# tenstack/batch-scheduler

Measured on NVIDIA H100. Metric: pod_x_node_fit_evals_per_sec, higher is better.
Workload: dtype int64

## Files before the change

batch-scheduler_b200/csrc/common.cuh:

```cuda
#pragma once
#include <cuda_runtime.h>
#include <stdint.h>

#include "../../include/bsched.h"

namespace bsk {

constexpr int LANE_CPU = 0, LANE_MEM = 1, LANE_EPH = 2, LANE_PODS = 3;
constexpr int64_t ABSENT_LEFT = (int64_t)1 << 61;
constexpr int64_t UNCHECKED_REQ = -((int64_t)1 << 61);
constexpr int32_t ABSENT_LEFT32 = 1 << 29;
constexpr int32_t UNCHECKED_REQ32 = -(1 << 29);
constexpr int FIT_CAP_LOG2 = 27;
constexpr int64_t NARROW_LIMIT = ((int64_t)1 << (FIT_CAP_LOG2 - 1)) - 1;
constexpr int32_t ABSENT_LEFTS = (1 << 30) - 1;
constexpr int32_t UNCHECKED_REQS = -((1 << 30) - 1);
constexpr int64_t SCALED_LIMIT = (int64_t)1 << 29;
struct LaneMap {
  uint8_t wide[BS_MAX_LANES];
  uint8_t narrow[BS_MAX_LANES];
  uint8_t scaled[BS_MAX_LANES];
  uint8_t sunit[BS_MAX_LANES];
  uint8_t sshift[BS_MAX_LANES];
  uint32_t sclamp[BS_MAX_LANES];
  uint32_t LW, LN, LS;
};
constexpr int NODE_TILE = 512;
constexpr int FIT_WARPS = 8;
constexpr int FIT_THREADS = (FIT_WARPS + 1) * 32;
constexpr int FIT_MIN_BLOCKS = 2;
constexpr int PODS_PER_WARP = 4;
constexpr int PODS_PER_CTA = FIT_WARPS * PODS_PER_WARP;
constexpr int TILE_WORDS = NODE_TILE / 32;
static_assert(TILE_WORDS <= 32 && 32 % TILE_WORDS == 0, "a 32-word bitmap line is a whole number of tiles");
constexpr int TILES_PER_LINE = 32 / TILE_WORDS;
constexpr int KEY_BITS = 4;
static_assert((1 << KEY_BITS) == TILE_WORDS, "the best-node key holds a word index of the tile in KEY_BITS bits");
static_assert(FIT_CAP_LOG2 + KEY_BITS <= 31, "best-node key: score (27 bits) + word index must fit 31 bits");
constexpr int FIT_STAGES = 2;
static_assert(TILE_WORDS % 4 == 0, "the fit kernel sweeps a tile 4 words at a time");
constexpr int FIT_NB = 2;
using ColBits = uint16_t;
static_assert(sizeof(ColBits) * 8 == TILE_WORDS, "one class bit per ballot word of a tile");

}
```

batch-scheduler_b200/csrc/fit.cuh:

```cuda
#pragma once
#include "common.cuh"

namespace bsk {

__device__ __forceinline__ uint32_t smem_u32(const void* p) {
  return (uint32_t)__cvta_generic_to_shared(p);
}
__device__ __forceinline__ void mbar_init(uint64_t* bar, uint32_t count) {
  asm volatile("mbarrier.init.shared::cta.b64 [%0], %1;" ::"r"(smem_u32(bar)), "r"(count));
}
__device__ __forceinline__ void mbar_expect_tx(uint64_t* bar, uint32_t bytes) {
  asm volatile("mbarrier.arrive.expect_tx.shared::cta.b64 _, [%0], %1;" ::"r"(smem_u32(bar)), "r"(bytes)
               : "memory");
}
__device__ __forceinline__ void mbar_arrive(uint64_t* bar) {
  asm volatile("mbarrier.arrive.shared::cta.b64 _, [%0];" ::"r"(smem_u32(bar)) : "memory");
}
__device__ __forceinline__ void mbar_wait(uint64_t* bar, uint32_t parity) {
  asm volatile(
      "{\n"
      ".reg .pred p;\n"
      "WAIT_%=:\n"
      "mbarrier.try_wait.parity.shared::cta.b64 p, [%0], %1;\n"
      "@p bra DONE_%=;\n"
      "bra WAIT_%=;\n"
      "DONE_%=:\n"
      "}\n" ::"r"(smem_u32(bar)),
      "r"(parity)
      : "memory");
}
__device__ __forceinline__ void tma_bulk_g2s(void* dst_smem, const void* src_gmem, uint32_t bytes,
                                             uint64_t* bar) {
  asm volatile(
      "cp.async.bulk.shared::cluster.global.mbarrier::complete_tx::bytes [%0], [%1], %2, [%3];" ::"r"(
          smem_u32(dst_smem)),
      "l"(src_gmem), "r"(bytes), "r"(smem_u32(bar))
      : "memory");
}
__device__ __forceinline__ uint64_t l2_evict_first() {
  uint64_t pol;
  asm volatile("createpolicy.fractional.L2::evict_first.b64 %0, 1.0;" : "=l"(pol));
  return pol;
}
__device__ __forceinline__ void tma_bulk_s2g(void* dst_gmem, uint32_t src_smem, uint32_t bytes, uint64_t pol) {
  asm volatile("cp.async.bulk.global.shared::cta.bulk_group.L2::cache_hint [%0], [%1], %2, %3;" ::"l"(dst_gmem),
               "r"(src_smem), "r"(bytes), "l"(pol)
               : "memory");
}
__device__ __forceinline__ void bulk_commit() { asm volatile("cp.async.bulk.commit_group;" ::: "memory"); }
template <int N>
__device__ __forceinline__ void bulk_wait_read() { asm volatile("cp.async.bulk.wait_group.read %0;" ::"n"(N) : "memory"); }
__device__ __forceinline__ void fence_async_smem() { asm volatile("fence.proxy.async.shared::cta;" ::: "memory"); }

__device__ __forceinline__ int64_t min64(int64_t a, int64_t b) { return a < b ? a : b; }
__device__ __forceinline__ int32_t hi32(int64_t v) {
  int32_t lo, hi;
  asm("mov.b64 {%0, %1}, %2;" : "=r"(lo), "=r"(hi) : "l"(v));
  (void)lo;
  return hi;
}
__device__ __forceinline__ uint32_t lo32(int64_t v) {
  int32_t lo, hi;
  asm("mov.b64 {%0, %1}, %2;" : "=r"(lo), "=r"(hi) : "l"(v));
  (void)hi;
  return (uint32_t)lo;
}
__device__ __forceinline__ void sts_u32(uint32_t saddr, uint32_t v) {
  asm volatile("st.shared.u32 [%0], %1;" ::"r"(saddr), "r"(v));
}
__device__ __forceinline__ void sts_v2u32(uint32_t saddr, uint32_t lo, uint32_t hi) {
  asm volatile("st.shared.v2.u32 [%0], {%1, %2};" ::"r"(saddr), "r"(lo), "r"(hi));
}
__device__ __forceinline__ void sts_u64(uint32_t saddr, long long v) {
  asm volatile("st.shared.u64 [%0], %1;" ::"r"(saddr), "l"(v));
}

struct FitArgs {
  const int64_t* left_w;
  const int32_t* left_n;
  const ColBits* classfit;
  const int64_t* req;
  const uint32_t* req_present;
  const uint32_t* fit_class;
  LaneMap lm;
  uint32_t* feasible_count;
  int32_t* best_node;
  int64_t* best_score;
  uint32_t* fit_bitmap;
  int64_t* score;
  uint64_t left_w_pitch, left_n_pitch;
  uint64_t score_pitch;
  uint32_t bitmap_pitch;
  uint32_t P, N, Npad, W;
  uint32_t n_full, tail_split;
  unsigned long long* best_packed;
  int32_t* topk_node;
  int64_t* topk_score;
  uint32_t topk_k;
};

template <bool NARROW> struct BestT { using type = int64_t; };
template <> struct BestT<true> { using type = int32_t; };

enum { FIT_OUT_NONE = 0, FIT_OUT_BITMAP = 1, FIT_OUT_SCORE = 2, FIT_OUT_TOPK = 3 };

template <typename S>
__device__ __forceinline__ S topk_insert(S* __restrict__ ls_p, int32_t* __restrict__ ln_p, uint32_t K, uint32_t cb,
                                         S s, int32_t n0 , uint32_t lane) {
  S ls = ls_p[lane];
  int32_t ln = ln_p[lane];
#pragma unroll 1
  do {
    const uint32_t src = __ffs(cb) - 1;
    cb &= cb - 1;
    const S cs = __shfl_sync(0xffffffffu, s, src);
    const int32_t cn = n0 + (int32_t)src;
    const uint32_t pos = __popc(__ballot_sync(0xffffffffu, ls > cs || (ls == cs && ln < cn)));
    if (pos < K) {
      const S us = __shfl_up_sync(0xffffffffu, ls, 1);
      const int32_t un = __shfl_up_sync(0xffffffffu, ln, 1);
      if (lane == pos) { ls = cs; ln = cn; }
      else if (lane > pos) { ls = us; ln = un; }
    }
  } while (cb);
  ls_p[lane] = ls;
  ln_p[lane] = ln;
  return __shfl_sync(0xffffffffu, ls, K - 1);
}

template <int LW, int LN, int LS, int OUT, int RN>
__device__ __forceinline__ void fit_tile(const FitArgs& a, const int64_t* __restrict__ tlw,
                                         const int32_t* __restrict__ tln,
                                         const int64_t (&rqw)[PODS_PER_WARP][LW > 0 ? LW : 1],
                                         const int32_t (&rqn)[PODS_PER_WARP][LN + LS > 0 ? LN + LS : 1],
                                         const ColBits (&colbits)[PODS_PER_WARP], int R0, uint32_t slab ,
                                         uint32_t* s_words, uint32_t wbase , uint32_t node_base, uint32_t lane,
                                         typename BestT<(LN > 0)>::type (&best_s)[PODS_PER_WARP],
                                         int32_t (&best_n)[PODS_PER_WARP], int32_t (&kb)[PODS_PER_WARP],
                                         uint32_t (&cnt)[PODS_PER_WARP],
                                         typename BestT<(LN > 0)>::type* tks, int32_t* tkn ,
                                         typename BestT<(LN > 0)>::type (&thr)[PODS_PER_WARP]) {
  constexpr bool SCORE = OUT == FIT_OUT_SCORE;
  constexpr bool TOPK = OUT == FIT_OUT_TOPK;
  constexpr bool WORDS = OUT == FIT_OUT_BITMAP || SCORE;
  using S = typename BestT<(LN > 0)>::type;
  static_assert(!SCORE || RN == 1, "a staging slab holds one matrix row");
  const int64_t* tpw = tlw + lane;
  const int32_t* tpn = tln + lane;
  int32_t node = (int32_t)(node_base + lane);
  uint32_t wp = smem_u32(s_words) + wbase * 4;
  uint32_t sp = slab + lane * 8;
  int32_t jrem = TILE_WORDS - 1;
#pragma unroll 1
  for (int jb = 0; jb < TILE_WORDS; jb += 4) {
#pragma unroll
    for (int jj = 0; jj < 4; ++jj) {
      int64_t lfw[LW > 0 ? LW : 1];
      int32_t lfn[LN + LS > 0 ? LN + LS : 1];
#pragma unroll
      for (int d = 0; d < LW; ++d) lfw[d] = tpw[d * NODE_TILE + jj * 32];
#pragma unroll
      for (int d = 0; d < LN + LS; ++d) lfn[d] = tpn[d * NODE_TILE + jj * 32];
#pragma unroll
      for (int i = 0; i < RN; ++i) {
        const int r = R0 + i;
        if (LN > 0) {
          int32_t t = lfn[0] - rqn[r][0];
#pragma unroll
          for (int d = 1; d < LN; ++d) t = min(t, lfn[d] - rqn[r][d]);
          uint32_t m32 = (uint32_t)t;
          int32_t sgn = t;
#pragma unroll
          for (int d = 0; d < LS; ++d) {
            const int32_t x = min(lfn[LN + d] - rqn[r][LN + d], (int32_t)a.lm.sclamp[d]);
            sgn |= x;
            m32 = min(m32, (uint32_t)x << a.lm.sshift[d]);
          }
#pragma unroll
          for (int d = 0; d < LW; ++d) {
            const int64_t w = lfw[d] - rqw[r][d];
            const int32_t whi = hi32(w);
            sgn |= whi;
            m32 = min(m32, whi != 0 ? 0xffffffffu : lo32(w));
          }
          const bool fit = (sgn >= 0) && ((colbits[r] >> (jb + jj)) & 1u);
          if (WORDS) sts_u32(wp + (r * 32 + jj) * 4, __ballot_sync(0xffffffffu, fit));
          else if (fit) ++cnt[r];
          if (TOPK && a.fit_bitmap) sts_u32(wp + (r * 32 + jj) * 4, __ballot_sync(0xffffffffu, fit));
          const int32_t key = (int32_t)(m32 << KEY_BITS) + (jrem - jj);
          if (!TOPK && fit) kb[r] = max(kb[r], key);
          if (SCORE) sts_v2u32(sp + jj * 32 * 8, fit ? m32 : 0u, fit ? 0u : 0x80000000u);
          if (TOPK) {
            const uint32_t cb = __ballot_sync(0xffffffffu, fit && (int32_t)m32 > thr[r]);
            if (cb) thr[r] = topk_insert<S>(tks + r * 32, tkn + r * 32, a.topk_k, cb, (int32_t)m32, node + jj * 32 - (int32_t)lane, lane);
          }
        } else {
          int64_t m = lfw[0] - rqw[r][0];
#pragma unroll
          for (int d = 1; d < LW; ++d) m = min64(m, lfw[d] - rqw[r][d]);
          const bool fit = (hi32(m) >= 0) && ((colbits[r] >> (jb + jj)) & 1u);
          if (WORDS) sts_u32(wp + (r * 32 + jj) * 4, __ballot_sync(0xffffffffu, fit));
          else if (fit) ++cnt[r];
          if (TOPK && a.fit_bitmap) sts_u32(wp + (r * 32 + jj) * 4, __ballot_sync(0xffffffffu, fit));
          if (!TOPK && fit && m > best_s[r]) { best_s[r] = m; best_n[r] = node + jj * 32; }
          if (SCORE) sts_u64(sp + jj * 32 * 8, fit ? (long long)m : (long long)INT64_MIN);
          if (TOPK) {
            const uint32_t cb = __ballot_sync(0xffffffffu, fit && m > thr[r]);
            if (cb) thr[r] = topk_insert<S>(tks + r * 32, tkn + r * 32, a.topk_k, cb, m, node + jj * 32 - (int32_t)lane, lane);
          }
        }
      }
    }
    tpw += 128;
    tpn += 128;
    node += 128;
    jrem -= 4;
    wp += 16;
    sp += 128 * 8;
  }
}

__host__ __device__ constexpr size_t fit_tile_bytes(int LW, int LN, int LS) {
  return (size_t)NODE_TILE * (8 * LW + 4 * (LN + LS));
}
__host__ __device__ constexpr size_t fit_slab_bytes() { return (size_t)NODE_TILE * 8; }
__host__ __device__ constexpr size_t fit_topk_bytes() { return (size_t)PODS_PER_CTA * BS_TOPK_MAX * 12; }
static_assert(BS_TOPK_MAX == 32, "a top-K list holds one entry per lane");
__host__ __device__ constexpr size_t fit_smem_front(int LW, int LN, int LS) {
  size_t b = FIT_STAGES * fit_tile_bytes(LW, LN, LS) + (size_t)PODS_PER_CTA * (8 * LW + 4 * (LN + LS));
  b = (b + 7) & ~(size_t)7;
  b += 2 * FIT_STAGES * sizeof(uint64_t) + (size_t)PODS_PER_CTA * 32 * sizeof(uint32_t);
  return (b + 127) & ~(size_t)127;
}
__host__ __device__ constexpr size_t fit_smem_total(int LW, int LN, int LS, int out) {
  return fit_smem_front(LW, LN, LS) + (out == FIT_OUT_SCORE  ? (size_t)FIT_WARPS * FIT_NB * fit_slab_bytes()
                                       : out == FIT_OUT_TOPK ? fit_topk_bytes()
                                                             : 0);
}
constexpr size_t FIT_SMEM_MAX = 227 * 1024;

template <int LW, int LN, int LS, int OUT>
__global__ void __launch_bounds__(FIT_THREADS, FIT_MIN_BLOCKS) gang_fit_kernel(FitArgs a) {
  constexpr bool SCORE = OUT == FIT_OUT_SCORE;
  constexpr bool TOPK = OUT == FIT_OUT_TOPK;
  constexpr bool WORDS = OUT == FIT_OUT_BITMAP || SCORE;
  extern __shared__ __align__(128) unsigned char smem_raw[];
  constexpr size_t STAGE_BYTES = fit_tile_bytes(LW, LN, LS);
  constexpr int LNS = LN + LS;
  unsigned char* s_tile = smem_raw;
  int64_t* s_req_w = reinterpret_cast<int64_t*>(smem_raw + FIT_STAGES * STAGE_BYTES);
  int32_t* s_req_n = reinterpret_cast<int32_t*>(s_req_w + PODS_PER_CTA * LW);
  uint64_t* s_bar = reinterpret_cast<uint64_t*>(
      (reinterpret_cast<uintptr_t>(s_req_n + PODS_PER_CTA * LNS) + 7) & ~(uintptr_t)7);
  uint64_t* s_full = s_bar;
  uint64_t* s_empty = s_bar + FIT_STAGES;
  uint32_t* s_words_all = reinterpret_cast<uint32_t*>(s_bar + 2 * FIT_STAGES);

  const uint32_t tid = threadIdx.x, lane = tid & 31, wid = tid >> 5;
  uint32_t* s_words = s_words_all + wid * PODS_PER_WARP * 32;
  uint32_t unit = blockIdx.x, piece = 0, npieces = 1;
  if (blockIdx.x >= a.n_full) {
    const uint32_t tl = blockIdx.x - a.n_full;
    unit = a.n_full + tl / a.tail_split;
    piece = tl % a.tail_split;
    npieces = a.tail_split;
  }
  const uint32_t pod0 = unit * PODS_PER_CTA;
  const uint32_t wpod0 = pod0 + wid * PODS_PER_WARP;
  const uint32_t n_tiles = a.Npad / NODE_TILE;
  const uint32_t n_lines = (n_tiles + TILES_PER_LINE - 1) / TILES_PER_LINE;
  const uint32_t tile_lo = min(n_tiles, (n_lines * piece / npieces) * TILES_PER_LINE);
  const uint32_t tile_hi = min(n_tiles, (n_lines * (piece + 1) / npieces) * TILES_PER_LINE);

  if (tid == 0) {
    for (int st = 0; st < FIT_STAGES; ++st) {
      mbar_init(&s_full[st], 1);
      mbar_init(&s_empty[st], FIT_WARPS);
    }
    asm volatile("fence.mbarrier_init.release.cluster;" ::: "memory");
  }
  for (uint32_t i = tid; i < PODS_PER_CTA * (LW + LNS); i += FIT_THREADS) {
    const uint32_t pl = i / (LW + LNS), k = i % (LW + LNS);
    const uint32_t p = pod0 + pl;
    const bool is_w = k < (uint32_t)LW;
    const uint32_t kn = k - LW;
    const uint32_t d = is_w ? a.lm.wide[k] : (kn < (uint32_t)LN ? a.lm.narrow[kn] : a.lm.scaled[kn - LN]);
    int64_t v = 0;
    bool present = true;
    if (p < a.P) {
      present = d < 4 || ((a.req_present[p] >> d) & 1u);
      v = present ? a.req[(size_t)d * a.P + p] : 0;
    }
    if (is_w) s_req_w[pl * LW + k] = present ? v : UNCHECKED_REQ;
    else if (kn < (uint32_t)LN) s_req_n[pl * LNS + kn] = present ? (int32_t)v : UNCHECKED_REQ32;
    else s_req_n[pl * LNS + kn] = present ? (int32_t)(v >> a.lm.sunit[kn - LN]) : UNCHECKED_REQS;
  }
  __syncthreads();
  auto issue = [&](uint32_t tile, uint32_t stage) {
    mbar_expect_tx(&s_full[stage], (uint32_t)STAGE_BYTES);
    unsigned char* dst = s_tile + stage * STAGE_BYTES;
    const unsigned char* src_w = reinterpret_cast<const unsigned char*>(a.left_w) + (uint64_t)tile * (NODE_TILE * 8);
    const unsigned char* src_n = reinterpret_cast<const unsigned char*>(a.left_n) + (uint64_t)tile * (NODE_TILE * 4);
#pragma unroll
    for (int d = 0; d < LW; ++d)
      tma_bulk_g2s(dst + (size_t)d * NODE_TILE * 8, src_w + (uint64_t)d * a.left_w_pitch, NODE_TILE * 8,
                   &s_full[stage]);
#pragma unroll
    for (int d = 0; d < LNS; ++d)
      tma_bulk_g2s(dst + (size_t)LW * NODE_TILE * 8 + (size_t)d * NODE_TILE * 4,
                   src_n + (uint64_t)d * a.left_n_pitch, NODE_TILE * 4, &s_full[stage]);
  };
  if (wid == FIT_WARPS) {
    if (lane == 0) {
      for (uint32_t tile = tile_lo; tile < tile_hi; ++tile) {
        const uint32_t st = (tile - tile_lo) % FIT_STAGES, use = (tile - tile_lo) / FIT_STAGES;
        if (use > 0) mbar_wait(&s_empty[st], (use - 1) & 1);
        issue(tile, st);
      }
    }
    return;
  }

  const bool want_bitmap = a.fit_bitmap != nullptr;
  uint32_t cnt[PODS_PER_WARP];
  typename BestT<(LN > 0)>::type best_s[PODS_PER_WARP];
  int32_t best_n[PODS_PER_WARP];
  int32_t kb[PODS_PER_WARP], kthr[PODS_PER_WARP];
  typename BestT<(LN > 0)>::type thr[PODS_PER_WARP];
  int64_t rqw[PODS_PER_WARP][LW > 0 ? LW : 1];
  int32_t rqn[PODS_PER_WARP][LNS > 0 ? LNS : 1];
  uint32_t coff[PODS_PER_WARP];
  typename BestT<(LN > 0)>::type* tks =
      reinterpret_cast<typename BestT<(LN > 0)>::type*>(smem_raw + fit_smem_front(LW, LN, LS)) + wid * PODS_PER_WARP * 32;
  int32_t* tkn = reinterpret_cast<int32_t*>(smem_raw + fit_smem_front(LW, LN, LS) + (size_t)PODS_PER_CTA * 32 * 8) +
                 wid * PODS_PER_WARP * 32;
#pragma unroll
  for (int r = 0; r < PODS_PER_WARP; ++r) {
    cnt[r] = 0; best_n[r] = -1; kb[r] = -1; kthr[r] = 0; thr[r] = -1;
    if (TOPK) { tks[r * 32 + lane] = -1; tkn[r * 32 + lane] = -1; }
    best_s[r] = LN > 0 ? (typename BestT<(LN > 0)>::type)(-1) : (typename BestT<(LN > 0)>::type)INT64_MIN;
    const uint32_t p = wpod0 + r;
    coff[r] = (p < a.P ? a.fit_class[p] : 0u) * n_tiles * 32 + lane;
#pragma unroll
    for (int d = 0; d < LW; ++d) rqw[r][d] = s_req_w[(wid * PODS_PER_WARP + r) * LW + d];
#pragma unroll
    for (int d = 0; d < LNS; ++d) rqn[r][d] = s_req_n[(wid * PODS_PER_WARP + r) * LNS + d];
  }
  const uint32_t slab0 = smem_u32(smem_raw + fit_smem_front(LW, LN, LS)) + wid * (uint32_t)(FIT_NB * fit_slab_bytes());
  int64_t* srow = SCORE ? a.score + (size_t)wpod0 * a.score_pitch : nullptr;

  uint32_t stage = 0, phase = 0, sb = 0, nseg = 0;
  ColBits colnext[PODS_PER_WARP];
#pragma unroll
  for (int r = 0; r < PODS_PER_WARP; ++r) colnext[r] = __ldg(a.classfit + coff[r] + min(tile_lo, n_tiles - 1) * 32);
  for (uint32_t tile = tile_lo; tile < tile_hi; ++tile) {
    ColBits colbits[PODS_PER_WARP];
    const uint32_t tnext = tile + 1 < tile_hi ? tile + 1 : tile;
#pragma unroll
    for (int r = 0; r < PODS_PER_WARP; ++r) {
      colbits[r] = colnext[r];
      colnext[r] = __ldg(a.classfit + coff[r] + tnext * 32);
    }
    mbar_wait(&s_full[stage], phase);
    const int64_t* tlw = reinterpret_cast<const int64_t*>(s_tile + stage * STAGE_BYTES);
    const int32_t* tln = reinterpret_cast<const int32_t*>(s_tile + stage * STAGE_BYTES + (size_t)LW * NODE_TILE * 8);
    const uint32_t node_base = tile * NODE_TILE;
    const uint32_t wbase = (tile % TILES_PER_LINE) * TILE_WORDS;
    if constexpr (SCORE) {
#pragma unroll
      for (int r = 0; r < PODS_PER_WARP; ++r) {
        const uint32_t slab = slab0 + sb * (uint32_t)fit_slab_bytes();
        if (nseg >= (uint32_t)FIT_NB) {
          if (lane == 0) bulk_wait_read<FIT_NB - 1>();
          __syncwarp();
        }
        fit_tile<LW, LN, LS, OUT, 1>(a, tlw, tln, rqw, rqn, colbits, r, slab, s_words, wbase, node_base, lane, best_s,
                                     best_n, kb, cnt, tks, tkn, thr);
        fence_async_smem();
        __syncwarp();
        if (lane == 0) {
          if (node_base < (uint32_t)a.score_pitch) {
            const uint32_t cols = min((uint32_t)NODE_TILE, (uint32_t)a.score_pitch - node_base);
            tma_bulk_s2g(srow + (size_t)r * a.score_pitch + node_base, slab, cols * 8, l2_evict_first());
          }
          bulk_commit();
        }
        ++nseg;
        if (++sb == FIT_NB) sb = 0;
      }
    } else {
      fit_tile<LW, LN, LS, OUT, PODS_PER_WARP>(a, tlw, tln, rqw, rqn, colbits, 0, 0, s_words, wbase, node_base, lane,
                                               best_s, best_n, kb, cnt, tks, tkn, thr);
    }
    if (LN > 0 && !TOPK) {
#pragma unroll
      for (int r = 0; r < PODS_PER_WARP; ++r) {
        if (kb[r] >= kthr[r]) {
          best_s[r] = kb[r] >> KEY_BITS;
          best_n[r] = (int32_t)(node_base + lane) + (TILE_WORDS - 1 - (kb[r] & (TILE_WORDS - 1))) * 32;
          kthr[r] = (best_s[r] + 1) << KEY_BITS;
        }
        kb[r] = -1;
      }
    }
    __syncwarp();
    if (lane == 0) mbar_arrive(&s_empty[stage]);
    if ((WORDS || (TOPK && want_bitmap)) && ((tile + 1) % TILES_PER_LINE == 0 || tile + 1 == tile_hi)) {
      const uint32_t line = tile / TILES_PER_LINE;
      const uint32_t valid = (tile % TILES_PER_LINE + 1) * TILE_WORDS;
      if (lane < valid) {
#pragma unroll
        for (int r = 0; r < PODS_PER_WARP; ++r) {
          const uint32_t w = s_words[r * 32 + lane];
          if (WORDS) cnt[r] += __popc(w);
          if (want_bitmap) a.fit_bitmap[(size_t)(wpod0 + r) * a.bitmap_pitch + line * 32 + lane] = w;
        }
      }
    }
    __syncwarp();
    if (++stage == FIT_STAGES) { stage = 0; phase ^= 1; }
  }
  if (SCORE && lane == 0) bulk_wait_read<0>();
  if (TOPK && lane < a.topk_k) {
#pragma unroll
    for (int r = 0; r < PODS_PER_WARP; ++r) {
      const size_t o = (size_t)(wpod0 + r) * a.topk_k + lane;
      const int32_t n = tkn[r * 32 + lane];
      a.topk_node[o] = n;
      a.topk_score[o] = n < 0 ? INT64_MIN : (int64_t)tks[r * 32 + lane];
    }
  }

#pragma unroll
  for (int k = 0; k < PODS_PER_WARP; ++k) {
    int32_t n = TOPK ? tkn[k * 32] : best_n[k];
    int64_t s = n < 0 ? INT64_MIN : TOPK ? (int64_t)tks[k * 32] : (int64_t)best_s[k];
    uint32_t c = cnt[k];
    for (int o = 16; o; o >>= 1) {
      const int64_t os = __shfl_xor_sync(0xffffffffu, s, o);
      const int32_t on = __shfl_xor_sync(0xffffffffu, n, o);
      c += __shfl_xor_sync(0xffffffffu, c, o);
      if (on >= 0 && (n < 0 || os > s || (os == s && on < n))) { s = os; n = on; }
    }
    const uint32_t p = wpod0 + k;
    if (p < a.P && lane == 0) {
      if (npieces == 1) {
        a.feasible_count[p] = c;
        a.best_node[p] = n;
        a.best_score[p] = s;
      } else {
        if (c) atomicAdd(&a.feasible_count[p], c);
        if (n >= 0) atomicMax(&a.best_packed[p], ((unsigned long long)(uint32_t)(s + 1) << 32) | (uint32_t)(~(uint32_t)n));
      }
    }
  }
}

static __global__ void fit_unpack_kernel(const unsigned long long* __restrict__ packed, uint32_t p0, uint32_t P,
                                         int32_t* __restrict__ best_node, int64_t* __restrict__ best_score) {
  const uint32_t p = p0 + blockIdx.x * blockDim.x + threadIdx.x;
  if (p >= P) return;
  const unsigned long long v = packed[p];
  if (v == 0) { best_node[p] = -1; best_score[p] = INT64_MIN; return; }
  best_node[p] = (int32_t)(~(uint32_t)v);
  best_score[p] = (int64_t)(v >> 32) - 1;
}
constexpr uint32_t FIT_TAIL_SPLIT = 8;

}

namespace bsk {
using FitFn = cudaError_t (*)(const FitArgs&, uint32_t units, cudaStream_t, uint32_t* launches, cudaEvent_t ev_a, cudaEvent_t ev_b);
constexpr int FIT_MAX_LN = 8;
constexpr int FIT_N_SLICES = FIT_MAX_LN + 1;
struct FitWS { int lw, ls; };
constexpr FitWS FIT_WS_COMBOS[] = {{0, 0}, {1, 0}, {2, 0}, {3, 0}, {4, 0}, {0, 1}, {0, 2}, {0, 3}, {1, 1}, {1, 2}, {2, 1}};
constexpr int FIT_N_WS = sizeof(FIT_WS_COMBOS) / sizeof(FIT_WS_COMBOS[0]);
inline bool fit_variant_exists(uint32_t LW, uint32_t LN, uint32_t LS) {
  if (LN == 0) return LS == 0 && LW >= 4 && LW <= BS_MAX_LANES;
  if (LN > (uint32_t)FIT_MAX_LN || LW + LN + LS < 4 || LW + LN + LS > BS_MAX_LANES) return false;
  for (int i = 0; i < FIT_N_WS; ++i)
    if ((uint32_t)FIT_WS_COMBOS[i].lw == LW && (uint32_t)FIT_WS_COMBOS[i].ls == LS) return true;
  return false;
}
FitFn fit_lookup_slice0(uint32_t LW, uint32_t LN, uint32_t LS, int out);
FitFn fit_lookup_slice1(uint32_t LW, uint32_t LN, uint32_t LS, int out);
FitFn fit_lookup_slice2(uint32_t LW, uint32_t LN, uint32_t LS, int out);
FitFn fit_lookup_slice3(uint32_t LW, uint32_t LN, uint32_t LS, int out);
FitFn fit_lookup_slice4(uint32_t LW, uint32_t LN, uint32_t LS, int out);
FitFn fit_lookup_slice5(uint32_t LW, uint32_t LN, uint32_t LS, int out);
FitFn fit_lookup_slice6(uint32_t LW, uint32_t LN, uint32_t LS, int out);
FitFn fit_lookup_slice7(uint32_t LW, uint32_t LN, uint32_t LS, int out);
FitFn fit_lookup_slice8(uint32_t LW, uint32_t LN, uint32_t LS, int out);
inline FitFn fit_lookup(uint32_t LW, uint32_t LN, uint32_t LS, int out) {
  switch (LN) {
    case 0: return fit_lookup_slice0(LW, LN, LS, out);
    case 1: return fit_lookup_slice1(LW, LN, LS, out);
    case 2: return fit_lookup_slice2(LW, LN, LS, out);
    case 3: return fit_lookup_slice3(LW, LN, LS, out);
    case 4: return fit_lookup_slice4(LW, LN, LS, out);
    case 5: return fit_lookup_slice5(LW, LN, LS, out);
    case 6: return fit_lookup_slice6(LW, LN, LS, out);
    case 7: return fit_lookup_slice7(LW, LN, LS, out);
    case 8: return fit_lookup_slice8(LW, LN, LS, out);
  }
  return nullptr;
}
}
```

batch-scheduler_b200/csrc/fit_inst.cu:

```cuda
#include <algorithm>

#include "fit.cuh"

#ifndef BS_FIT_SLICE
#error "compile with -DBS_FIT_SLICE=<0..8>"
#endif

namespace bsk {
namespace {

template <int LW, int LN, int LS, int OUT>
cudaError_t launch_fit_t(const FitArgs& a0, uint32_t units, cudaStream_t s, uint32_t* launches, cudaEvent_t ev_a, cudaEvent_t ev_b) {
  constexpr size_t smem = fit_smem_total(LW, LN, LS, OUT);
  static_assert(smem <= FIT_SMEM_MAX, "the fit kernel's shared memory exceeds what one CTA may use");
  cudaError_t er = cudaFuncSetAttribute(gang_fit_kernel<LW, LN, LS, OUT>, cudaFuncAttributeMaxDynamicSharedMemorySize,
                                        (int)smem);
  if (er != cudaSuccess) return er;
  FitArgs a = a0;
  a.n_full = units;
  a.tail_split = 1;
  if (LN > 0 && OUT != FIT_OUT_TOPK && a.best_packed && units) {
    int per_sm = 0, dev = 0, sms = 0;
    if (cudaOccupancyMaxActiveBlocksPerMultiprocessor(&per_sm, gang_fit_kernel<LW, LN, LS, OUT>, FIT_THREADS, smem) == cudaSuccess &&
        cudaGetDevice(&dev) == cudaSuccess && cudaDeviceGetAttribute(&sms, cudaDevAttrMultiProcessorCount, dev) == cudaSuccess &&
        per_sm > 0 && sms > 0) {
      const uint32_t slots = (uint32_t)per_sm * (uint32_t)sms;
      const uint32_t n_tiles = a.Npad / NODE_TILE, n_lines = (n_tiles + TILES_PER_LINE - 1) / TILES_PER_LINE;
      const uint32_t n_full = units / slots * slots, tail = units - n_full;
      const uint32_t split = std::min<uint32_t>(FIT_TAIL_SPLIT, n_lines);
      if (tail && split > 1 && tail * 10 < slots * 9) {
        a.n_full = n_full;
        a.tail_split = split;
      }
    }
  }
  const uint32_t tail_units = units - a.n_full;
  if (a.tail_split > 1) {
    const uint32_t p0 = a.n_full * PODS_PER_CTA;
    if (p0 < a.P) {
      er = cudaMemsetAsync(a.feasible_count + p0, 0, (size_t)(a.P - p0) * 4, s);
      if (er == cudaSuccess) er = cudaMemsetAsync(a.best_packed + p0, 0, (size_t)(a.P - p0) * 8, s);
      if (er != cudaSuccess) return er;
    }
  }
  if (ev_a) cudaEventRecord(ev_a, s);
  gang_fit_kernel<LW, LN, LS, OUT><<<a.n_full + tail_units * a.tail_split, FIT_THREADS, smem, s>>>(a);
  if (ev_b) cudaEventRecord(ev_b, s);
  if (launches) *launches = 1;
  if (a.tail_split > 1) {
    const uint32_t p0 = a.n_full * PODS_PER_CTA;
    if (p0 < a.P) {
      fit_unpack_kernel<<<(a.P - p0 + 255) / 256, 256, 0, s>>>(a.best_packed, p0, a.P, a.best_node, a.best_score);
      if (launches) *launches = 2;
    }
  }
  return cudaGetLastError();
}

template <int LW, int LN, int LS>
FitFn pick(int out) {
  switch (out) {
    case FIT_OUT_SCORE: return launch_fit_t<LW, LN, LS, FIT_OUT_SCORE>;
    case FIT_OUT_BITMAP: return launch_fit_t<LW, LN, LS, FIT_OUT_BITMAP>;
    case FIT_OUT_TOPK: return launch_fit_t<LW, LN, LS, FIT_OUT_TOPK>;
  }
  return launch_fit_t<LW, LN, LS, FIT_OUT_NONE>;
}

}

#define BS_CAT2(a, b) a##b
#define BS_CAT(a, b) BS_CAT2(a, b)

FitFn BS_CAT(fit_lookup_slice, BS_FIT_SLICE)(uint32_t LW, uint32_t LN, uint32_t LS, int score) {
#if BS_FIT_SLICE == 0
  if (LN != 0 || LS != 0) return nullptr;
  switch (LW) {
    case 4: return pick<4, 0, 0>(score);
    case 6: return pick<6, 0, 0>(score);
    case 7: return pick<7, 0, 0>(score);
    case 8: return pick<8, 0, 0>(score);
    case 9: return pick<9, 0, 0>(score);
    case 10: return pick<10, 0, 0>(score);
    case 11: return pick<11, 0, 0>(score);
    case 12: return pick<12, 0, 0>(score);
    case 13: return pick<13, 0, 0>(score);
    case 14: return pick<14, 0, 0>(score);
    case 15: return pick<15, 0, 0>(score);
    case 16: return pick<16, 0, 0>(score);
    case 5: return pick<5, 0, 0>(score);
  }
  return nullptr;
#else
  constexpr int N = BS_FIT_SLICE;
  if (LN != (uint32_t)N || !fit_variant_exists(LW, LN, LS)) return nullptr;
  const uint32_t key = LW * 8 + LS;
  switch (key) {
#define BS_CASE(lw, ls)                                                        \
  case lw * 8 + ls:                                                            \
    if constexpr (lw + N + ls >= 4) return pick<lw, N, ls>(score); else break;
    BS_CASE(0, 0) BS_CASE(1, 0) BS_CASE(2, 0) BS_CASE(3, 0) BS_CASE(4, 0) BS_CASE(0, 1) BS_CASE(0, 2) BS_CASE(0, 3)
    BS_CASE(1, 1) BS_CASE(1, 2) BS_CASE(2, 1)
#undef BS_CASE
  }
  return nullptr;
#endif
}

}
```

profiles/microbench/store_pattern2.cu:

```cuda
#include <cstdio>
#include <cstdint>
#include <cstring>
#include <cuda_runtime.h>

__device__ __forceinline__ uint32_t smem_u32(const void* p) { return (uint32_t)__cvta_generic_to_shared(p); }
__device__ __forceinline__ void bulk_s2g(void* gdst, const void* ssrc, uint32_t bytes) {
  asm volatile("cp.async.bulk.global.shared::cta.bulk_group [%0], [%1], %2;" ::"l"(gdst), "r"(smem_u32(ssrc)), "r"(bytes)
               : "memory");
}
__device__ __forceinline__ void bulk_commit() { asm volatile("cp.async.bulk.commit_group;" ::: "memory"); }
template <int N>
__device__ __forceinline__ void bulk_wait_read() { asm volatile("cp.async.bulk.wait_group.read %0;" ::"n"(N) : "memory"); }
__device__ __forceinline__ void fence_async_smem() { asm volatile("fence.proxy.async.shared::cta;" ::: "memory"); }

__global__ void fill(long long* p, size_t n) {
  for (size_t i = blockIdx.x * (size_t)blockDim.x + threadIdx.x; i < n; i += (size_t)gridDim.x * blockDim.x) __stcs(p + i, 7ll);
}

template <int R>
__global__ void rows(long long* out, int P, int N) {
  const int lane = threadIdx.x & 31, wid = threadIdx.x >> 5, nw = blockDim.x >> 5;
  const int row0 = (blockIdx.x * nw + wid) * R;
  for (int base = 0; base < N; base += 512)
    for (int j = 0; j < 16; ++j)
#pragma unroll
      for (int r = 0; r < R; ++r) {
        const int n = base + j * 32 + lane;
        if (row0 + r < P && n < N) __stcs(out + (size_t)(row0 + r) * N + n, (long long)(n + r));
      }
}

template <int R>
__global__ void rowsv2(long long* out, int P, int N) {
  const int lane = threadIdx.x & 31, wid = threadIdx.x >> 5, nw = blockDim.x >> 5;
  const int row0 = (blockIdx.x * nw + wid) * R;
  for (int base = 0; base < N; base += 512)
    for (int j = 0; j < 8; ++j)
#pragma unroll
      for (int r = 0; r < R; ++r) {
        const int n = base + j * 64 + lane * 2;
        if (row0 + r < P && n + 1 < N)
          __stcs(reinterpret_cast<longlong2*>(out + (size_t)(row0 + r) * N + n), make_longlong2(n + r, n + r + 1));
      }
}

template <int R, int T, int NB, int WARPS>
__global__ void __launch_bounds__(WARPS * 32) tma(long long* out, int P, int N) {
  extern __shared__ __align__(128) unsigned char smem[];
  const int lane = threadIdx.x & 31, wid = threadIdx.x >> 5;
  long long* slab = reinterpret_cast<long long*>(smem) + (size_t)wid * NB * R * T;
  const int row0 = (blockIdx.x * WARPS + wid) * R;
  if (row0 >= P) return;
  int it = 0;
  for (int base = 0; base < N; base += T, ++it) {
    long long* s = slab + (size_t)(it % NB) * R * T;
    if (it >= NB) {
      if (lane == 0) bulk_wait_read<NB - 1>();
      __syncwarp();
    }
    const int cols = min(T, N - base);
#pragma unroll 4
    for (int j = 0; j < T / 32; ++j)
#pragma unroll
      for (int r = 0; r < R; ++r) s[r * T + j * 32 + lane] = (long long)(base + j * 32 + lane + r);
    fence_async_smem();
    __syncwarp();
    if (lane == 0) {
#pragma unroll
      for (int r = 0; r < R; ++r)
        if (row0 + r < P) bulk_s2g(out + (size_t)(row0 + r) * N + base, s + r * T, (uint32_t)cols * 8);
      bulk_commit();
    }
  }
  if (lane == 0) bulk_wait_read<0>();
}

template <int R, int T, int NB, int WARPS>
__global__ void __launch_bounds__(WARPS * 32) tmacta(long long* out, int P, int N) {
  extern __shared__ __align__(128) unsigned char smem[];
  const int lane = threadIdx.x & 31, wid = threadIdx.x >> 5;
  constexpr int ROWS = R * WARPS;
  long long* slab0 = reinterpret_cast<long long*>(smem);
  const int row0 = blockIdx.x * ROWS;
  int it = 0;
  for (int base = 0; base < N; base += T, ++it) {
    long long* s = slab0 + (size_t)(it % NB) * ROWS * T;
    if (it >= NB) {
      if (threadIdx.x == 0) bulk_wait_read<NB - 1>();
      __syncthreads();
    }
    const int cols = min(T, N - base);
#pragma unroll 4
    for (int j = 0; j < T / 32; ++j)
#pragma unroll
      for (int r = 0; r < R; ++r) s[(wid * R + r) * T + j * 32 + lane] = (long long)(base + j * 32 + lane + r);
    fence_async_smem();
    __syncthreads();
    if (threadIdx.x == 0) {
      for (int r = 0; r < ROWS; ++r)
        if (row0 + r < P) bulk_s2g(out + (size_t)(row0 + r) * N + base, s + r * T, (uint32_t)cols * 8);
      bulk_commit();
    }
  }
  if (threadIdx.x == 0) bulk_wait_read<0>();
}

template <class F>
float timeit(F f) {
  cudaEvent_t a, b;
  cudaEventCreate(&a); cudaEventCreate(&b);
  for (int i = 0; i < 3; ++i) f();
  float best = 1e9f, sum = 0;
  for (int i = 0; i < 10; ++i) {
    cudaEventRecord(a); f(); cudaEventRecord(b); cudaEventSynchronize(b);
    float ms; cudaEventElapsedTime(&ms, a, b); best = ms < best ? ms : best; sum += ms;
  }
  cudaEventDestroy(a); cudaEventDestroy(b);
  printf("   [avg %.3f]", sum / 10);
  return best;
}

static long long* d;
static const int P = 100000, N = 10000;
static void rep(const char* name, float ms) {
  cudaError_t e = cudaGetLastError();
  printf(" %-28s %.3f ms  %.0f GB/s  %s\n", name, ms, (double)P * N * 8 / ms / 1e6, e == cudaSuccess ? "" : cudaGetErrorString(e));
}

template <int R, int T, int NB, int WARPS>
void run_tma(const char* name, size_t smem_pad = 0) {
  const size_t smem = smem_pad ? smem_pad : (size_t)WARPS * NB * R * T * 8;
  cudaFuncSetAttribute(tma<R, T, NB, WARPS>, cudaFuncAttributeMaxDynamicSharedMemorySize, (int)smem);
  int occ = 0;
  cudaOccupancyMaxActiveBlocksPerMultiprocessor(&occ, tma<R, T, NB, WARPS>, WARPS * 32, smem);
  const int grid = (P + R * WARPS - 1) / (R * WARPS);
  cudaMemset(d, 0xff, 1 << 20);
  float ms = timeit([&] { tma<R, T, NB, WARPS><<<grid, WARPS * 32, smem>>>(d, P, N); });
  long long h[4];
  cudaMemcpy(h, d + 5, 8, cudaMemcpyDeviceToHost);
  cudaMemcpy(h + 1, d + (size_t)(R > 1 ? 1 : 0) * N + 9999, 8, cudaMemcpyDeviceToHost);
  cudaMemcpy(h + 2, d + (size_t)(P - 1) * N + 4097, 8, cudaMemcpyDeviceToHost);
  const bool ok = h[0] == 5 && h[1] == 9999 + (R > 1 ? 1 : 0) && h[2] == 4097 + ((P - 1) % R);
  char buf[96];
  snprintf(buf, sizeof buf, "%s occ=%d smem=%zuK %s", name, occ, smem >> 10, ok ? "ok" : "BAD");
  rep(buf, ms);
}
template <int R, int T, int NB, int WARPS>
void run_tmacta(const char* name) {
  const size_t smem = (size_t)WARPS * NB * R * T * 8;
  cudaFuncSetAttribute(tmacta<R, T, NB, WARPS>, cudaFuncAttributeMaxDynamicSharedMemorySize, (int)smem);
  int occ = 0;
  cudaOccupancyMaxActiveBlocksPerMultiprocessor(&occ, tmacta<R, T, NB, WARPS>, WARPS * 32, smem);
  const int grid = (P + R * WARPS - 1) / (R * WARPS);
  float ms = timeit([&] { tmacta<R, T, NB, WARPS><<<grid, WARPS * 32, smem>>>(d, P, N); });
  long long h[4];
  cudaMemcpy(h, d + 5, 8, cudaMemcpyDeviceToHost);
  cudaMemcpy(h + 2, d + (size_t)(P - 1) * N + 4097, 8, cudaMemcpyDeviceToHost);
  const bool ok = h[0] == 5 && h[2] == 4097 + ((P - 1) % R);
  char buf[96];
  snprintf(buf, sizeof buf, "%s occ=%d smem=%zuK %s", name, occ, smem >> 10, ok ? "ok" : "BAD");
  rep(buf, ms);
}

int main(int argc, char** argv) {
  const size_t n = (size_t)P * N;
  cudaMalloc(&d, n * 8 + (1 << 20));
  if (argc > 1 && !strcmp(argv[1], "occ2")) {
    constexpr size_t FIT_SMEM = 90880;
    for (int k = 0; k < 3; ++k) {
      run_tma<4, 128, 2, 8>("tma R4 T128 NB2 W8 pad", FIT_SMEM);
      run_tma<1, 512, 2, 8>("tma R1 T512 NB2 W8 pad", FIT_SMEM);
      run_tma<2, 256, 2, 8>("tma R2 T256 NB2 W8 pad", FIT_SMEM);
    }
    rep("memset", timeit([&] { cudaMemsetAsync(d, 1, n * 8); }));
    cudaError_t e = cudaDeviceSynchronize();
    printf("status: %s\n", cudaGetErrorString(e));
    return 0;
  }
  rep("fill", timeit([&] { fill<<<132 * 8, 256>>>(d, n); }));
  rep("memset", timeit([&] { cudaMemsetAsync(d, 1, n * 8); }));
  rep("rows<4> (round-1 pattern)", timeit([&] { rows<4><<<(P + 31) / 32, 256>>>(d, P, N); }));
  rep("rows<1> 8 rows/CTA", timeit([&] { rows<1><<<(P + 7) / 8, 256>>>(d, P, N); }));
  rep("rows<1> 16 rows/CTA", timeit([&] { rows<1><<<(P + 15) / 16, 512>>>(d, P, N); }));
  rep("rowsv2<4> 16B stores", timeit([&] { rowsv2<4><<<(P + 31) / 32, 256>>>(d, P, N); }));
  rep("rowsv2<1> 16B stores", timeit([&] { rowsv2<1><<<(P + 7) / 8, 256>>>(d, P, N); }));
  run_tma<4, 128, 2, 8>("tma R4 T128 NB2 W8");
  run_tma<4, 256, 2, 8>("tma R4 T256 NB2 W8");
  run_tma<4, 512, 1, 8>("tma R4 T512 NB1 W8");
  run_tma<2, 256, 2, 8>("tma R2 T256 NB2 W8");
  run_tma<2, 512, 2, 8>("tma R2 T512 NB2 W8");
  run_tma<1, 512, 2, 8>("tma R1 T512 NB2 W8");
  run_tma<1, 1024, 2, 8>("tma R1 T1024 NB2 W8");
  run_tma<4, 256, 3, 4>("tma R4 T256 NB3 W4");
  run_tma<4, 128, 4, 8>("tma R4 T128 NB4 W8");
  run_tma<4, 64, 4, 8>("tma R4 T64 NB4 W8");
  run_tmacta<4, 128, 2, 8>("tmacta R4 T128 NB2 W8");
  run_tmacta<4, 256, 2, 8>("tmacta R4 T256 NB2 W8");
  run_tmacta<4, 64, 3, 8>("tmacta R4 T64 NB3 W8");
  cudaError_t e = cudaDeviceSynchronize();
  printf("status: %s\n", cudaGetErrorString(e));
  return 0;
}
```

Measured before the change: 353.4 billion.

## Give score-mode fit warps one pod each and launch four times more CTAs

In score-output mode each warp now handles a single pod instead of four, so a CTA covers 8 pods and the grid is scaled up to match. Each warp streams one contiguous matrix row through its staging slabs instead of interleaving four rows per node tile. The aim is more CTAs and warps sharing the score-matrix store bandwidth, with long sequential bulk stores per row. In exchange, every node tile is loaded into shared memory four times as often across the grid, since fewer pods reuse each staged tile. A microbenchmark comparing the two row-store patterns is also added.

```diff
diff --git a/batch-scheduler_b200/csrc/common.cuh b/batch-scheduler_b200/csrc/common.cuh
--- a/batch-scheduler_b200/csrc/common.cuh
+++ b/batch-scheduler_b200/csrc/common.cuh
@@ -31,6 +31,9 @@
 constexpr int FIT_MIN_BLOCKS = 2;
 constexpr int PODS_PER_WARP = 4;
 constexpr int PODS_PER_CTA = FIT_WARPS * PODS_PER_WARP;
+constexpr int SCORE_PODS_PER_WARP = 1;
+constexpr int SCORE_PODS_PER_CTA = FIT_WARPS * SCORE_PODS_PER_WARP;
+static_assert(PODS_PER_CTA % SCORE_PODS_PER_CTA == 0, "score-mode CTAs tile the padded rows");
 constexpr int TILE_WORDS = NODE_TILE / 32;
 static_assert(TILE_WORDS <= 32 && 32 % TILE_WORDS == 0, "a 32-word bitmap line is a whole number of tiles");
 constexpr int TILES_PER_LINE = 32 / TILE_WORDS;
diff --git a/batch-scheduler_b200/csrc/fit.cuh b/batch-scheduler_b200/csrc/fit.cuh
--- a/batch-scheduler_b200/csrc/fit.cuh
+++ b/batch-scheduler_b200/csrc/fit.cuh
@@ -128,23 +128,23 @@
   return __shfl_sync(0xffffffffu, ls, K - 1);
 }
 
-template <int LW, int LN, int LS, int OUT, int RN>
+template <int LW, int LN, int LS, int OUT, int PW>
 __device__ __forceinline__ void fit_tile(const FitArgs& a, const int64_t* __restrict__ tlw,
                                          const int32_t* __restrict__ tln,
-                                         const int64_t (&rqw)[PODS_PER_WARP][LW > 0 ? LW : 1],
-                                         const int32_t (&rqn)[PODS_PER_WARP][LN + LS > 0 ? LN + LS : 1],
-                                         const ColBits (&colbits)[PODS_PER_WARP], int R0, uint32_t slab ,
+                                         const int64_t (&rqw)[PW][LW > 0 ? LW : 1],
+                                         const int32_t (&rqn)[PW][LN + LS > 0 ? LN + LS : 1],
+                                         const ColBits (&colbits)[PW], uint32_t slab ,
                                          uint32_t* s_words, uint32_t wbase , uint32_t node_base, uint32_t lane,
-                                         typename BestT<(LN > 0)>::type (&best_s)[PODS_PER_WARP],
-                                         int32_t (&best_n)[PODS_PER_WARP], int32_t (&kb)[PODS_PER_WARP],
-                                         uint32_t (&cnt)[PODS_PER_WARP],
+                                         typename BestT<(LN > 0)>::type (&best_s)[PW],
+                                         int32_t (&best_n)[PW], int32_t (&kb)[PW],
+                                         uint32_t (&cnt)[PW],
                                          typename BestT<(LN > 0)>::type* tks, int32_t* tkn ,
-                                         typename BestT<(LN > 0)>::type (&thr)[PODS_PER_WARP]) {
+                                         typename BestT<(LN > 0)>::type (&thr)[PW]) {
   constexpr bool SCORE = OUT == FIT_OUT_SCORE;
   constexpr bool TOPK = OUT == FIT_OUT_TOPK;
   constexpr bool WORDS = OUT == FIT_OUT_BITMAP || SCORE;
   using S = typename BestT<(LN > 0)>::type;
-  static_assert(!SCORE || RN == 1, "a staging slab holds one matrix row");
+  static_assert(!SCORE || PW == 1, "a staging slab holds one matrix row");
   const int64_t* tpw = tlw + lane;
   const int32_t* tpn = tln + lane;
   int32_t node = (int32_t)(node_base + lane);
@@ -162,8 +162,7 @@
 #pragma unroll
       for (int d = 0; d < LN + LS; ++d) lfn[d] = tpn[d * NODE_TILE + jj * 32];
 #pragma unroll
-      for (int i = 0; i < RN; ++i) {
-        const int r = R0 + i;
+      for (int r = 0; r < PW; ++r) {
         if (LN > 0) {
           int32_t t = lfn[0] - rqn[r][0];
 #pragma unroll
@@ -238,12 +237,15 @@
                                                              : 0);
 }
 constexpr size_t FIT_SMEM_MAX = 227 * 1024;
+__host__ __device__ constexpr int fit_pods_per_warp(int out) { return out == FIT_OUT_SCORE ? SCORE_PODS_PER_WARP : PODS_PER_WARP; }
+__host__ __device__ constexpr int fit_pods_per_cta(int out) { return FIT_WARPS * fit_pods_per_warp(out); }
 
 template <int LW, int LN, int LS, int OUT>
 __global__ void __launch_bounds__(FIT_THREADS, FIT_MIN_BLOCKS) gang_fit_kernel(FitArgs a) {
   constexpr bool SCORE = OUT == FIT_OUT_SCORE;
   constexpr bool TOPK = OUT == FIT_OUT_TOPK;
   constexpr bool WORDS = OUT == FIT_OUT_BITMAP || SCORE;
+  constexpr int PPW = fit_pods_per_warp(OUT), PPC = fit_pods_per_cta(OUT);
   extern __shared__ __align__(128) unsigned char smem_raw[];
   constexpr size_t STAGE_BYTES = fit_tile_bytes(LW, LN, LS);
   constexpr int LNS = LN + LS;
@@ -257,7 +259,7 @@
   uint32_t* s_words_all = reinterpret_cast<uint32_t*>(s_bar + 2 * FIT_STAGES);
 
   const uint32_t tid = threadIdx.x, lane = tid & 31, wid = tid >> 5;
-  uint32_t* s_words = s_words_all + wid * PODS_PER_WARP * 32;
+  uint32_t* s_words = s_words_all + wid * PPW * 32;
   uint32_t unit = blockIdx.x, piece = 0, npieces = 1;
   if (blockIdx.x >= a.n_full) {
     const uint32_t tl = blockIdx.x - a.n_full;
@@ -265,8 +267,8 @@
     piece = tl % a.tail_split;
     npieces = a.tail_split;
   }
-  const uint32_t pod0 = unit * PODS_PER_CTA;
-  const uint32_t wpod0 = pod0 + wid * PODS_PER_WARP;
+  const uint32_t pod0 = unit * PPC;
+  const uint32_t wpod0 = pod0 + wid * PPW;
   const uint32_t n_tiles = a.Npad / NODE_TILE;
   const uint32_t n_lines = (n_tiles + TILES_PER_LINE - 1) / TILES_PER_LINE;
   const uint32_t tile_lo = min(n_tiles, (n_lines * piece / npieces) * TILES_PER_LINE);
@@ -279,7 +281,7 @@
     }
     asm volatile("fence.mbarrier_init.release.cluster;" ::: "memory");
   }
-  for (uint32_t i = tid; i < PODS_PER_CTA * (LW + LNS); i += FIT_THREADS) {
+  for (uint32_t i = tid; i < PPC * (LW + LNS); i += FIT_THREADS) {
     const uint32_t pl = i / (LW + LNS), k = i % (LW + LNS);
     const uint32_t p = pod0 + pl;
     const bool is_w = k < (uint32_t)LW;
@@ -322,42 +324,42 @@
   }
 
   const bool want_bitmap = a.fit_bitmap != nullptr;
-  uint32_t cnt[PODS_PER_WARP];
-  typename BestT<(LN > 0)>::type best_s[PODS_PER_WARP];
-  int32_t best_n[PODS_PER_WARP];
-  int32_t kb[PODS_PER_WARP], kthr[PODS_PER_WARP];
-  typename BestT<(LN > 0)>::type thr[PODS_PER_WARP];
-  int64_t rqw[PODS_PER_WARP][LW > 0 ? LW : 1];
-  int32_t rqn[PODS_PER_WARP][LNS > 0 ? LNS : 1];
-  uint32_t coff[PODS_PER_WARP];
+  uint32_t cnt[PPW];
+  typename BestT<(LN > 0)>::type best_s[PPW];
+  int32_t best_n[PPW];
+  int32_t kb[PPW], kthr[PPW];
+  typename BestT<(LN > 0)>::type thr[PPW];
+  int64_t rqw[PPW][LW > 0 ? LW : 1];
+  int32_t rqn[PPW][LNS > 0 ? LNS : 1];
+  uint32_t coff[PPW];
   typename BestT<(LN > 0)>::type* tks =
       reinterpret_cast<typename BestT<(LN > 0)>::type*>(smem_raw + fit_smem_front(LW, LN, LS)) + wid * PODS_PER_WARP * 32;
   int32_t* tkn = reinterpret_cast<int32_t*>(smem_raw + fit_smem_front(LW, LN, LS) + (size_t)PODS_PER_CTA * 32 * 8) +
                  wid * PODS_PER_WARP * 32;
 #pragma unroll
-  for (int r = 0; r < PODS_PER_WARP; ++r) {
+  for (int r = 0; r < PPW; ++r) {
     cnt[r] = 0; best_n[r] = -1; kb[r] = -1; kthr[r] = 0; thr[r] = -1;
     if (TOPK) { tks[r * 32 + lane] = -1; tkn[r * 32 + lane] = -1; }
     best_s[r] = LN > 0 ? (typename BestT<(LN > 0)>::type)(-1) : (typename BestT<(LN > 0)>::type)INT64_MIN;
     const uint32_t p = wpod0 + r;
     coff[r] = (p < a.P ? a.fit_class[p] : 0u) * n_tiles * 32 + lane;
 #pragma unroll
-    for (int d = 0; d < LW; ++d) rqw[r][d] = s_req_w[(wid * PODS_PER_WARP + r) * LW + d];
-#pragma unroll
-    for (int d = 0; d < LNS; ++d) rqn[r][d] = s_req_n[(wid * PODS_PER_WARP + r) * LNS + d];
+    for (int d = 0; d < LW; ++d) rqw[r][d] = s_req_w[(wid * PPW + r) * LW + d];
+#pragma unroll
+    for (int d = 0; d < LNS; ++d) rqn[r][d] = s_req_n[(wid * PPW + r) * LNS + d];
   }
   const uint32_t slab0 = smem_u32(smem_raw + fit_smem_front(LW, LN, LS)) + wid * (uint32_t)(FIT_NB * fit_slab_bytes());
   int64_t* srow = SCORE ? a.score + (size_t)wpod0 * a.score_pitch : nullptr;
 
   uint32_t stage = 0, phase = 0, sb = 0, nseg = 0;
-  ColBits colnext[PODS_PER_WARP];
-#pragma unroll
-  for (int r = 0; r < PODS_PER_WARP; ++r) colnext[r] = __ldg(a.classfit + coff[r] + min(tile_lo, n_tiles - 1) * 32);
+  ColBits colnext[PPW];
+#pragma unroll
+  for (int r = 0; r < PPW; ++r) colnext[r] = __ldg(a.classfit + coff[r] + min(tile_lo, n_tiles - 1) * 32);
   for (uint32_t tile = tile_lo; tile < tile_hi; ++tile) {
-    ColBits colbits[PODS_PER_WARP];
+    ColBits colbits[PPW];
     const uint32_t tnext = tile + 1 < tile_hi ? tile + 1 : tile;
 #pragma unroll
-    for (int r = 0; r < PODS_PER_WARP; ++r) {
+    for (int r = 0; r < PPW; ++r) {
       colbits[r] = colnext[r];
       colnext[r] = __ldg(a.classfit + coff[r] + tnext * 32);
     }
@@ -367,34 +369,31 @@
     const uint32_t node_base = tile * NODE_TILE;
     const uint32_t wbase = (tile % TILES_PER_LINE) * TILE_WORDS;
     if constexpr (SCORE) {
-#pragma unroll
-      for (int r = 0; r < PODS_PER_WARP; ++r) {
-        const uint32_t slab = slab0 + sb * (uint32_t)fit_slab_bytes();
-        if (nseg >= (uint32_t)FIT_NB) {
-          if (lane == 0) bulk_wait_read<FIT_NB - 1>();
-          __syncwarp();
+      const uint32_t slab = slab0 + sb * (uint32_t)fit_slab_bytes();
+      if (nseg >= (uint32_t)FIT_NB) {
+        if (lane == 0) bulk_wait_read<FIT_NB - 1>();
+        __syncwarp();
+      }
+      fit_tile<LW, LN, LS, OUT, PPW>(a, tlw, tln, rqw, rqn, colbits, slab, s_words, wbase, node_base, lane, best_s,
+                                     best_n, kb, cnt, tks, tkn, thr);
+      fence_async_smem();
+      __syncwarp();
+      if (lane == 0) {
+        if (node_base < (uint32_t)a.score_pitch) {
+          const uint32_t cols = min((uint32_t)NODE_TILE, (uint32_t)a.score_pitch - node_base);
+          tma_bulk_s2g(srow + node_base, slab, cols * 8, l2_evict_first());
         }
-        fit_tile<LW, LN, LS, OUT, 1>(a, tlw, tln, rqw, rqn, colbits, r, slab, s_words, wbase, node_base, lane, best_s,
-                                     best_n, kb, cnt, tks, tkn, thr);
-        fence_async_smem();
-        __syncwarp();
-        if (lane == 0) {
-          if (node_base < (uint32_t)a.score_pitch) {
-            const uint32_t cols = min((uint32_t)NODE_TILE, (uint32_t)a.score_pitch - node_base);
-            tma_bulk_s2g(srow + (size_t)r * a.score_pitch + node_base, slab, cols * 8, l2_evict_first());
-          }
-          bulk_commit();
-        }
-        ++nseg;
-        if (++sb == FIT_NB) sb = 0;
-      }
+        bulk_commit();
+      }
+      ++nseg;
+      if (++sb == FIT_NB) sb = 0;
     } else {
-      fit_tile<LW, LN, LS, OUT, PODS_PER_WARP>(a, tlw, tln, rqw, rqn, colbits, 0, 0, s_words, wbase, node_base, lane,
-                                               best_s, best_n, kb, cnt, tks, tkn, thr);
+      fit_tile<LW, LN, LS, OUT, PPW>(a, tlw, tln, rqw, rqn, colbits, 0, s_words, wbase, node_base, lane, best_s, best_n,
+                                     kb, cnt, tks, tkn, thr);
     }
     if (LN > 0 && !TOPK) {
 #pragma unroll
-      for (int r = 0; r < PODS_PER_WARP; ++r) {
+      for (int r = 0; r < PPW; ++r) {
         if (kb[r] >= kthr[r]) {
           best_s[r] = kb[r] >> KEY_BITS;
           best_n[r] = (int32_t)(node_base + lane) + (TILE_WORDS - 1 - (kb[r] & (TILE_WORDS - 1))) * 32;
@@ -410,7 +409,7 @@
       const uint32_t valid = (tile % TILES_PER_LINE + 1) * TILE_WORDS;
       if (lane < valid) {
 #pragma unroll
-        for (int r = 0; r < PODS_PER_WARP; ++r) {
+        for (int r = 0; r < PPW; ++r) {
           const uint32_t w = s_words[r * 32 + lane];
           if (WORDS) cnt[r] += __popc(w);
           if (want_bitmap) a.fit_bitmap[(size_t)(wpod0 + r) * a.bitmap_pitch + line * 32 + lane] = w;
@@ -423,7 +422,7 @@
   if (SCORE && lane == 0) bulk_wait_read<0>();
   if (TOPK && lane < a.topk_k) {
 #pragma unroll
-    for (int r = 0; r < PODS_PER_WARP; ++r) {
+    for (int r = 0; r < PPW; ++r) {
       const size_t o = (size_t)(wpod0 + r) * a.topk_k + lane;
       const int32_t n = tkn[r * 32 + lane];
       a.topk_node[o] = n;
@@ -432,7 +431,7 @@
   }
 
 #pragma unroll
-  for (int k = 0; k < PODS_PER_WARP; ++k) {
+  for (int k = 0; k < PPW; ++k) {
     int32_t n = TOPK ? tkn[k * 32] : best_n[k];
     int64_t s = n < 0 ? INT64_MIN : TOPK ? (int64_t)tks[k * 32] : (int64_t)best_s[k];
     uint32_t c = cnt[k];
diff --git a/batch-scheduler_b200/csrc/fit_inst.cu b/batch-scheduler_b200/csrc/fit_inst.cu
--- a/batch-scheduler_b200/csrc/fit_inst.cu
+++ b/batch-scheduler_b200/csrc/fit_inst.cu
@@ -16,6 +16,8 @@
   cudaError_t er = cudaFuncSetAttribute(gang_fit_kernel<LW, LN, LS, OUT>, cudaFuncAttributeMaxDynamicSharedMemorySize,
                                         (int)smem);
   if (er != cudaSuccess) return er;
+  constexpr uint32_t PPC = fit_pods_per_cta(OUT);
+  units = std::min(units * (uint32_t)(PODS_PER_CTA / PPC), (a0.P + PPC - 1) / PPC);
   FitArgs a = a0;
   a.n_full = units;
   a.tail_split = 1;
@@ -36,7 +38,7 @@
   }
   const uint32_t tail_units = units - a.n_full;
   if (a.tail_split > 1) {
-    const uint32_t p0 = a.n_full * PODS_PER_CTA;
+    const uint32_t p0 = a.n_full * PPC;
     if (p0 < a.P) {
       er = cudaMemsetAsync(a.feasible_count + p0, 0, (size_t)(a.P - p0) * 4, s);
       if (er == cudaSuccess) er = cudaMemsetAsync(a.best_packed + p0, 0, (size_t)(a.P - p0) * 8, s);
@@ -48,7 +50,7 @@
   if (ev_b) cudaEventRecord(ev_b, s);
   if (launches) *launches = 1;
   if (a.tail_split > 1) {
-    const uint32_t p0 = a.n_full * PODS_PER_CTA;
+    const uint32_t p0 = a.n_full * PPC;
     if (p0 < a.P) {
       fit_unpack_kernel<<<(a.P - p0 + 255) / 256, 256, 0, s>>>(a.best_packed, p0, a.P, a.best_node, a.best_score);
       if (launches) *launches = 2;
diff --git a/profiles/microbench/store_pattern2.cu b/profiles/microbench/store_pattern2.cu
--- a/profiles/microbench/store_pattern2.cu
+++ b/profiles/microbench/store_pattern2.cu
@@ -70,6 +70,35 @@
       for (int r = 0; r < R; ++r)
         if (row0 + r < P) bulk_s2g(out + (size_t)(row0 + r) * N + base, s + r * T, (uint32_t)cols * 8);
       bulk_commit();
+    }
+  }
+  if (lane == 0) bulk_wait_read<0>();
+}
+
+template <int RW, int T, int NB, int WARPS>
+__global__ void __launch_bounds__(WARPS * 32) tmarr(long long* out, int P, int N) {
+  extern __shared__ __align__(128) unsigned char smem[];
+  const int lane = threadIdx.x & 31, wid = threadIdx.x >> 5;
+  long long* slab = reinterpret_cast<long long*>(smem) + (size_t)wid * NB * T;
+  const int row0 = (blockIdx.x * WARPS + wid) * RW;
+  if (row0 >= P) return;
+  int it = 0;
+  for (int base = 0; base < N; base += T) {
+    const int cols = min(T, N - base);
+    for (int r = 0; r < RW; ++r, ++it) {
+      long long* s = slab + (size_t)(it % NB) * T;
+      if (it >= NB) {
+        if (lane == 0) bulk_wait_read<NB - 1>();
+        __syncwarp();
+      }
+#pragma unroll 4
+      for (int j = 0; j < T / 32; ++j) s[j * 32 + lane] = (long long)(base + j * 32 + lane + r);
+      fence_async_smem();
+      __syncwarp();
+      if (lane == 0) {
+        if (row0 + r < P) bulk_s2g(out + (size_t)(row0 + r) * N + base, s, (uint32_t)cols * 8);
+        bulk_commit();
+      }
     }
   }
   if (lane == 0) bulk_wait_read<0>();
@@ -145,6 +174,24 @@
   snprintf(buf, sizeof buf, "%s occ=%d smem=%zuK %s", name, occ, smem >> 10, ok ? "ok" : "BAD");
   rep(buf, ms);
 }
+template <int RW, int T, int NB, int WARPS>
+void run_tmarr(const char* name, size_t smem_pad) {
+  const size_t smem = smem_pad;
+  cudaFuncSetAttribute(tmarr<RW, T, NB, WARPS>, cudaFuncAttributeMaxDynamicSharedMemorySize, (int)smem);
+  int occ = 0;
+  cudaOccupancyMaxActiveBlocksPerMultiprocessor(&occ, tmarr<RW, T, NB, WARPS>, WARPS * 32, smem);
+  const int grid = (P + RW * WARPS - 1) / (RW * WARPS);
+  cudaMemset(d, 0xff, 1 << 20);
+  float ms = timeit([&] { tmarr<RW, T, NB, WARPS><<<grid, WARPS * 32, smem>>>(d, P, N); });
+  long long h[4];
+  cudaMemcpy(h, d + 5, 8, cudaMemcpyDeviceToHost);
+  cudaMemcpy(h + 1, d + (size_t)N + 9999, 8, cudaMemcpyDeviceToHost);
+  cudaMemcpy(h + 2, d + (size_t)(P - 1) * N + 4097, 8, cudaMemcpyDeviceToHost);
+  const bool ok = h[0] == 5 && h[1] == 9999 + 1 && h[2] == 4097 + ((P - 1) % RW);
+  char buf[96];
+  snprintf(buf, sizeof buf, "%s occ=%d smem=%zuK %s", name, occ, smem >> 10, ok ? "ok" : "BAD");
+  rep(buf, ms);
+}
 template <int R, int T, int NB, int WARPS>
 void run_tmacta(const char* name) {
   const size_t smem = (size_t)WARPS * NB * R * T * 8;
@@ -165,8 +212,18 @@
 int main(int argc, char** argv) {
   const size_t n = (size_t)P * N;
   cudaMalloc(&d, n * 8 + (1 << 20));
+  constexpr size_t FIT_SMEM = 90880;
+  if (argc > 1 && !strcmp(argv[1], "occ2rr")) {
+    for (int k = 0; k < 3; ++k) {
+      run_tmarr<4, 512, 2, 8>("tmarr RW4 T512 NB2 W8 pad", FIT_SMEM);
+      run_tma<1, 512, 2, 8>("tma R1 T512 NB2 W8 pad", FIT_SMEM);
+    }
+    rep("memset", timeit([&] { cudaMemsetAsync(d, 1, n * 8); }));
+    cudaError_t e = cudaDeviceSynchronize();
+    printf("status: %s\n", cudaGetErrorString(e));
+    return 0;
+  }
   if (argc > 1 && !strcmp(argv[1], "occ2")) {
-    constexpr size_t FIT_SMEM = 90880;
     for (int k = 0; k < 3; ++k) {
       run_tma<4, 128, 2, 8>("tma R4 T128 NB2 W8 pad", FIT_SMEM);
       run_tma<1, 512, 2, 8>("tma R1 T512 NB2 W8 pad", FIT_SMEM);
```

After: 360.1 billion (median of 6 runs). 1.9% higher.
